# matthieugomez/LeastSquaresOptim.jl

Measured on AMD Instinct MI355X. Metric: lm_lsmr_outer_iterations_per_sec, higher is better.
Workload: dtype f64

## Files before the change

include/lsqhip.h:

```cpp
#ifndef LSQHIP_H
#define LSQHIP_H
#include <stddef.h>
#ifdef __cplusplus
extern "C" {
#endif

typedef enum {
    LSQ_OK = 0,
    LSQ_EDIM = 1,
    LSQ_ENOTPD = 2,
    LSQ_ERANK = 3,
    LSQ_ENONFINITE = 4,
    LSQ_EBOUNDS = 5,
    LSQ_EHIP = 6,
    LSQ_EARG = 7,
    LSQ_ECALLBACK = 8,
    LSQ_ERCCL = 9
} lsq_status;

typedef struct lsq_ctx lsq_ctx;
typedef struct lsq_mat lsq_mat;
typedef struct lsq_solver lsq_solver;
typedef struct lsq_model lsq_model;

// ... 128 lines not shown
    int bad_index;
    double seconds;
    long long lsmr_iterations;
    double ssr0;
} lsq_result;

void lsq_options_default(lsq_options *opt);
int lsq_optimize(lsq_ctx *ctx, int optimizer, int solver_kind, lsq_mat *J, double *d_x,
                 double *d_fcur, lsq_f_callback f, lsq_g_callback g, void *user,
                 const lsq_options *opt, lsq_result *res);

typedef struct {
    double *ssr, *ssr0;
    int *iterations;
    int *converged, *x_converged, *f_converged, *g_converged;
    int *f_calls, *g_calls, *mul_calls;
    int *status, *info;
    int outer_iterations;
    double seconds;
    int trace_cap;
    double *trace_ssr, *trace_gnorm, *trace_delta, *trace_rho;
    int *trace_accept;
    double *trace_x;
} lsq_batched_result;
int lsq_optimize_batched(lsq_ctx *ctx, int optimizer, int solver_kind, lsq_mat *J, double *d_x,
                         double *d_fcur, lsq_f_callback f, lsq_g_callback g, void *user,
                         const lsq_options *opt, void *batched_result);

int lsq_model_tanh_create(lsq_ctx *ctx, lsq_mat *J, const double *h_Avalues, const double *h_b,
                          lsq_model **out);
int lsq_model_destroy(lsq_model *md);
lsq_f_callback lsq_model_f(void);
lsq_g_callback lsq_model_g(void);

int lsq_synth_sparse(int m, int n, int per_col, unsigned long long seed, int *h_colptr,
                     int *h_rowval, double *h_nzval);
int lsq_synth_dense(int m, int n, unsigned long long seed, double *h_values);
int lsq_synth_uniform(int n, unsigned long long seed, double lo, double hi, double *h_out);
int lsq_synth_normal(int n, unsigned long long seed, double *h_out);

int lsq_bench_mul(lsq_mat *J, int trans, int reps, const double *d_x, double *d_y, double beta,
                  float *h_ms_per_launch);

int lsq_bench_occupy(lsq_ctx *ctx, int workgroups, int lds_bytes, double milliseconds);
int lsq_bench_occupy_wait(lsq_ctx *ctx);

int lsq_set_exact(int on);

int lsq_debug_set(int launch_jitter_us, int serial);
int lsq_debug_get(int *launch_jitter_us, int *serial, long long *stalls);

int lsq_prof_begin(lsq_ctx *ctx, int max_samples);
int lsq_prof_select(lsq_ctx *ctx, int kernel_mask);
int lsq_prof_end(lsq_ctx *ctx, double h_avg_ms[2], int h_count[2]);
int lsq_prof_overhead(lsq_ctx *ctx, int pairs, double *h_ms);

#ifdef __cplusplus
}
#endif
#endif
```

leastsquaresoptim.jl_amd/_lib.py:

```python
import ctypes as C
import os
import re
import subprocess

_HERE = os.path.dirname(os.path.abspath(__file__))
ROOT = os.path.dirname(_HERE)
LIB_PATH = os.environ.get("LSQ_LIB_PATH") or os.path.join(_HERE, "liblsqhip.so")
HEADER = os.path.join(ROOT, "include", "lsqhip.h")

c_dp = C.POINTER(C.c_double)
c_ip = C.POINTER(C.c_int)

F_CALLBACK = C.CFUNCTYPE(C.c_int, C.c_void_p, C.c_void_p, C.c_void_p)
G_CALLBACK = C.CFUNCTYPE(C.c_int, C.c_void_p, C.c_void_p, C.c_void_p)
ALLREDUCE_CALLBACK = C.CFUNCTYPE(C.c_int, c_dp, C.c_int, C.c_void_p)
OP_MUL_CALLBACK = C.CFUNCTYPE(C.c_int, C.c_int, C.c_void_p, C.c_void_p, C.c_void_p)
OP_COLSUM_CALLBACK = C.CFUNCTYPE(C.c_int, C.c_void_p, C.c_void_p)
PRECOND_CALLBACK = C.CFUNCTYPE(C.c_int, C.c_void_p, C.c_void_p, C.c_void_p, C.c_void_p)
ROW_ALLREDUCE_CALLBACK = C.CFUNCTYPE(C.c_int, C.c_void_p, C.c_int, C.c_void_p, C.c_void_p)
PRECOND_UPDATE_CALLBACK = C.CFUNCTYPE(C.c_int, C.c_void_p, C.c_void_p, C.c_void_p)
PRECOND_LDIV_CALLBACK = C.CFUNCTYPE(C.c_int, C.c_void_p, C.c_void_p, C.c_void_p)

OK, EDIM, ENOTPD, ERANK, ENONFINITE, EBOUNDS, EHIP, EARG, ECALLBACK, ERCCL = range(10)
QR, CHOLESKY, LSMR, BLOCK_QR = 0, 1, 2, 3
# ... 113 lines not shown
        "lsq_clamp": (i, [vp, i, d, d, vp]),
        "lsq_ediv": (i, [vp, i, vp, vp, vp]),
        "lsq_box_clip": (i, [vp, i, vp, vp, vp, vp]),
        "lsq_first_nonfinite": (i, [vp, i, vp, c_ip]),
        "lsq_solver_create": (i, [vp, vp, i, i, pvp]),
        "lsq_solver_destroy": (i, [vp]),
        "lsq_ldiv": (i, [vp, vp, vp, vp, c_ip]),
        "lsq_ldiv_damped": (i, [vp, vp, vp, vp, vp, c_ip]),
        "lsq_solver_set_row_allreduce": (i, [vp, ROW_ALLREDUCE_CALLBACK, vp, C.c_longlong]),
        "lsq_solver_info": (i, [vp, c_ip, c_ip, c_ip]),
        "lsq_solver_qr_path": (i, [vp, c_ip]),
        "lsq_solver_qr_panel": (i, [vp, c_ip]),
        "lsq_solver_chol_path": (i, [vp, c_ip]),
        "lsq_solver_lsmr_path": (i, [vp, c_ip]),
        "lsq_solver_blockdiag_path": (i, [vp, c_ip, c_ip]),
        "lsq_solver_blockdiag_ranks": (i, [vp, c_ip]),
        "lsq_solver_covariance": (i, [vp, vp, vp, vp, vp, c_ip]),
        "lsq_dense_covariance": (i, [vp, vp, vp, vp, vp, c_ip]),
        "lsq_solver_stats": (i, [vp, c_ip, c_ip]),
        "lsq_ctx_fallback_stats": (i, [vp, c_ip]),
        "lsq_ctx_device_info": (i, [vp, c_ip, c_ip, C.c_char_p, i]),
        "lsq_ctx_tail_stats": (i, [vp, C.POINTER(C.c_longlong)]),
        "lsq_bench_occupy": (i, [vp, i, i, d]),
        "lsq_bench_occupy_wait": (i, [vp]),
        "lsq_options_default": (None, [C.POINTER(Options)]),
        "lsq_optimize": (i, [vp, i, i, vp, vp, vp, F_CALLBACK, G_CALLBACK, vp, C.POINTER(Options),
                             C.POINTER(Result)]),
        "lsq_optimize_batched": (i, [vp, i, i, vp, vp, vp, F_CALLBACK, G_CALLBACK, vp, C.POINTER(Options),
                                     C.POINTER(BatchedResult)]),
        "lsq_model_tanh_create": (i, [vp, vp, c_dp, c_dp, pvp]),
        "lsq_model_destroy": (i, [vp]),
        "lsq_model_f": (F_CALLBACK, []),
        "lsq_model_g": (G_CALLBACK, []),
        "lsq_synth_sparse": (i, [i, i, i, C.c_ulonglong, c_ip, c_ip, c_dp]),
        "lsq_synth_dense": (i, [i, i, C.c_ulonglong, c_dp]),
        "lsq_synth_uniform": (i, [i, C.c_ulonglong, d, d, c_dp]),
        "lsq_synth_normal": (i, [i, C.c_ulonglong, c_dp]),
        "lsq_set_exact": (i, [i]),
        "lsq_debug_set": (i, [i, i]),
        "lsq_debug_get": (i, [c_ip, c_ip, C.POINTER(C.c_longlong)]),
        "lsq_prof_begin": (i, [vp, i]),
        "lsq_prof_select": (i, [vp, i]),
        "lsq_prof_end": (i, [vp, c_dp, c_ip]),
        "lsq_prof_overhead": (i, [vp, i, c_dp]),
        "lsq_bench_mul": (i, [vp, i, i, vp, vp, d, C.POINTER(C.c_float)]),
    }
    for name, (res, args) in sig.items():
        fn = getattr(L, name)
        fn.restype = res
        fn.argtypes = args
    L._signatures = sig
    _LIB = L
    return L


class LsqError(RuntimeError):

    def __init__(self, status, msg):
        super().__init__(msg)
        self.status = status


class DimensionMismatch(LsqError):
    pass


# ... 34 lines not shown
```

leastsquaresoptim.jl_amd/csrc/lsq_optimize.hip:

```cpp
#include <chrono>
#include <cmath>
#include <cstring>

#include "lsq_solver.h"
#include "lsq_spmv.h"

static constexpr double MIN_DELTA = 1e-16, MAX_DELTA = 1e16, MIN_STEP_QUALITY = 1e-3;
static constexpr double MIN_DIAGONAL = 1e-6, MAX_DIAGONAL = 1e32;
static constexpr double DECREASE_THRESHOLD = 0.25, INCREASE_THRESHOLD = 0.75;

enum { SL_GRAD = 8, SL_DX = 9, SL_NONFIN = 10, SL_TRIAL = 11, SL_PRED = 12, SL_SSR = 13, SL_W0 = 14, SL_W1 = 15,
       SL_W2 = 16, SL_SUM = 17 };

extern "C" int lsq_solver_create(lsq_ctx *c, lsq_mat *J, int kind, int for_lm, lsq_solver **out) {
    LSQ_RANGE("lsq_solver_create");
    if (!c || !J || !out) return LSQ_EARG;
    if (kind == LSQ_QR && J->kind != LSQ_MAT_DENSE) {
        lsq_set_error("solver QR() is not available for sparse Jacobians. Choose between Cholesky() and LSMR()");
        return LSQ_EARG;
    }
    const bool blockdiag = kind == LSQ_CHOLESKY && J->kind == LSQ_MAT_CSC && J->bd_blocks > 0;
    const bool bordered = kind == LSQ_CHOLESKY && J->kind == LSQ_MAT_CSC && J->br_blocks > 0;
    if (kind == LSQ_CHOLESKY && J->kind != LSQ_MAT_DENSE && !blockdiag && !bordered) {
        lsq_set_error("MethodError: no AbstractAllocatedSolver for Cholesky() with a sparse Jacobian "
// ... 1155 lines not shown
            res->status = LSQ_EARG;
            return LSQ_EARG;
        }
        LSQ_TRY(lsq_solver_set_row_allreduce(w->solver, opt->row_allreduce, opt->row_allreduce_user,
                                             opt->global_rows > 0 ? opt->global_rows : (long long)J->m));
    } else if (w->solver->kind == LSQ_LSMR) {
        LSQ_TRY(lsq_solver_set_row_allreduce(w->solver, nullptr, nullptr, 0));
    }
    auto t0 = std::chrono::steady_clock::now();
    int st = lm ? optimize_lm(c, w->solver, *w->buf, J, x, fcur, f, g, user, opt, res)
                : optimize_dogleg(c, w->solver, *w->buf, J, x, fcur, f, g, user, opt, res);
    hipStreamSynchronize(c->stream);
    res->seconds = std::chrono::duration<double>(std::chrono::steady_clock::now() - t0).count();
    res->status = st;
    return st;
}

struct lsq_model {
    lsq_ctx *ctx;
    lsq_mat *J;
    bool fused = false;
    double *d_Acsc = nullptr;
    double *d_Acsr = nullptr;
    double *d_Ab = nullptr;
    double *d_b = nullptr;
    double *d_t = nullptr;
    double *d_s = nullptr;
    double *d_sspec = nullptr;
    const double *tanh_x = nullptr;
    const double *sfac_x = nullptr;
    double *d_b_perm = nullptr;
    double *d_perm[2] = {nullptr, nullptr};
    const double *perm_of[2] = {nullptr, nullptr};
};
static void model_perm_invalidate(lsq_model *md, const double *vec) {
    for (int k = 0; k < 2; ++k)
        if (!vec || md->perm_of[k] == vec) md->perm_of[k] = nullptr;
}

__global__ void __launch_bounds__(LSQ_NT) k_tanh(int n, const double *__restrict__ x, double *__restrict__ t) {
    for (int i = blockIdx.x * LSQ_NT + threadIdx.x; i < n; i += gridDim.x * LSQ_NT) t[i] = tanh(x[i]);
}

struct EpiResidual {
    static constexpr bool REDUCE = false;
    const int *done;
    int extra_blocks;
    const double *b;
    double *out;
    double *partials;
    unsigned *counter;
    __device__ void seg(int i, double dot, double &) const { out[i] = dot - b[i]; }
    using has_pre = void;
    __device__ double pre(int i) const { return b[i]; }
    __device__ void seg_pre(int i, double dot, double bi, double &) const { out[i] = dot - bi; }
    __device__ void extra(int, double &) const {}
    __device__ void finalize(double) const {}
};

struct EpiResidualSq {
    static constexpr bool REDUCE = true;
    const int *done;
    int extra_blocks;
    const double *b;
    double *out;
    double *partials;
// ... 230 lines not shown
    return hipGetLastError() == hipSuccess ? 0 : 1;
}

static int model_pair_tail(void *user, lsq_mat *J, const double *dx, const double *fcur, double *ftrial, const double *xt,
                           double *slot_pred, double *slot_trial, LsqSlotPublish pub, const int *skip, bool *done, SpecGrad *sg) {
    lsq_model *md = (lsq_model *)user;
    lsq_ctx *c = md->ctx;
    *done = false;
    if (!(model_pair_applies(md, J) && md->tanh_x == xt)) return 0;
    const LsqSell &S = J->srows;
    const int nxpad = (J->n + 1) & ~1;
    const size_t lds = (size_t)std::max(2 * nxpad, LSQ_SELL_ROWS_MAX) * sizeof(double);
    if (lsq_set_lds(c, (const void *)k_sell_rows_pair<0>, (size_t)2 * LSQ_PAIR_X_MAX * sizeof(double)) != LSQ_OK) return 0;
    const size_t plen = (size_t)S.nslices * 64;
    const int pgrid = std::max(1, std::min(lsq_div_up((long long)plen, LSQ_NT), c->num_cus * 8));
    if (!model_perm_ready(md)) return 0;
    int k = md->perm_of[0] == fcur ? 0 : (md->perm_of[1] == fcur ? 1 : -1);
    if (k < 0) {
        k = 0;
        LSQ_LAUNCH(k_sell_perm_rows<0>, dim3(pgrid), dim3(LSQ_NT), 0, c->stream, sell_dev(S), S.wrows, S.nslices, fcur, md->d_perm[k]);
        md->perm_of[k] = fcur;
    }
    md->perm_of[1 - k] = ftrial;
    md->tanh_x = nullptr;
    const int grid = std::max(1, std::min(S.nblocks, c->num_cus));
    const bool spec = sg && sg->gate && md->sfac_x == xt;
    SellPairEpi e{skip, md->d_perm[k], md->d_b_perm, ftrial, md->d_perm[1 - k], c->d_partials, c->d_partials + 4096, lsq_ctr(c, 7),
                  slot_pred, slot_trial, pub, spec ? sg->gate : nullptr, spec ? sg->ssr : 0.0, MIN_STEP_QUALITY,
                  c->d_slots + SL_SSR, c->d_slots + SL_DX, c->d_slots + SL_GRAD, spec ? sg->xtol : 0.0, spec ? sg->ftol : 0.0,
                  spec ? sg->gtol : 0.0};
    LSQ_LAUNCH(k_sell_rows_pair<0>, dim3(grid), dim3(LSQ_BIG_NT), lds, c->stream, sell_dev(S), S.wrows, J->m, dx, J->d_colscale,
               (const double *)md->d_t, J->n, nxpad, e);
    *done = true;
    if (hipGetLastError() != hipSuccess) return 1;
    if (spec) {
        const int st = lsq_sparse_grad_colsum_spec(J, ftrial, sg->grad, md->d_sspec, sg->gate);
        if (st == LSQ_OK) sg->launched = true;
        else if (st != LSQ_EARG) return 1;
    }
    return 0;
}

static int model_g(lsq_mat *J, const double *x, void *user) {
    lsq_model *md = (lsq_model *)user;
    lsq_ctx *c = md->ctx;
    if (J->kind == LSQ_MAT_DENSE) {}
    else if (md->sfac_x == x) std::swap(md->d_s, md->d_sspec);
    else LSQ_LAUNCH(k_sfac, dim3(ngrid(c, J->n)), dim3(LSQ_NT), 0, c->stream, J->n, x, md->d_s);
    md->sfac_x = nullptr;
    md->tanh_x = nullptr;
    if (md->fused) {
        if (lsq_mat_set_colscale(J, md->d_s) != LSQ_OK) return 1;
        return hipGetLastError() == hipSuccess ? 0 : 1;
    }
    if (J->kind == LSQ_MAT_CSC) {
        const bool have_cols = J->scols.active || J->nwin > 1;
        const unsigned short *rcol = J->srows.active ? J->srows.d_idx16 : J->csr.d_idx16;
        const unsigned short *ccol = J->scols.active ? J->scols.d_col16 : J->bcsc.d_col16;
        double *rval = J->srows.active ? J->srows.d_val : J->csr.d_val;
        double *cval = J->scols.active ? J->scols.d_val : J->bcsc.d_val;
        const long long rlen = lsq_mirror_rows_len(J), clen = lsq_mirror_cols_len(J);
        const bool lds_ok = J->n <= 12000 && J->nnz >= (1 << 20) && J->srows.ncw == 1;
        const bool lazy_csc = lds_ok && rcol && have_cols && ccol && lsq_can_fuse_grad_colsum(J);
        if (!lazy_csc) {
            int grid = J->n < c->num_cus * 16 ? (J->n > 0 ? J->n : 1) : c->num_cus * 16;
            LSQ_LAUNCH(k_scale_cols, dim3(grid), dim3(LSQ_NT), 0, c->stream, J->n, J->csc.d_ptr, 0, md->d_Acsc,
// ... 64 lines not shown
    LSQ_HIP(hipMalloc(&md->d_t, nb));
    LSQ_HIP(hipMalloc(&md->d_s, nb));
    LSQ_HIP(hipMalloc(&md->d_sspec, nb));
    if (lsq_colscale_fusable(J)) {
        LSQ_TRY(lsq_mat_set_values(J, hA));
        LSQ_TRY(lsq_fill(c, J->n, 1.0, md->d_s));
        LSQ_TRY(lsq_mat_set_colscale(J, md->d_s));
        md->fused = true;
        LSQ_HIP(hipStreamSynchronize(c->stream));
        *out = md;
        return LSQ_OK;
    }
    size_t vb = (size_t)(J->nnz + 8) * sizeof(double);
    LSQ_HIP(hipMalloc(&md->d_Acsc, vb));
    LSQ_ZERO(md->d_Acsc, 0, vb);
    LSQ_HIP(hipMemcpy(md->d_Acsc, hA, (size_t)J->nnz * sizeof(double), hipMemcpyHostToDevice));
    if (J->kind == LSQ_MAT_CSC) {
        const size_t rb = (size_t)(lsq_mirror_rows_len(J) + 1024) * sizeof(double);
        LSQ_HIP(hipMalloc(&md->d_Acsr, rb));
        LSQ_ZERO(md->d_Acsr, 0, rb);
        LSQ_TRY(lsq_mirror_rows(J, md->d_Acsc, md->d_Acsr));
        if (lsq_mirror_cols_len(J) > 0) {
            const size_t cbytes = (size_t)(lsq_mirror_cols_len(J) + 1024) * sizeof(double);
            LSQ_HIP(hipMalloc(&md->d_Ab, cbytes));
            LSQ_ZERO(md->d_Ab, 0, cbytes);
            LSQ_TRY(lsq_mirror_cols(J, md->d_Acsc, md->d_Ab));
        }
        LSQ_HIP(hipStreamSynchronize(c->stream));
    }
    *out = md;
    return LSQ_OK;
}

extern "C" int lsq_model_destroy(lsq_model *md) {
    if (!md) return LSQ_OK;
    hipStreamSynchronize(md->ctx->stream);
    if (md->fused && md->J) lsq_mat_set_colscale(md->J, nullptr);
    hipFree(md->d_Acsc); hipFree(md->d_Acsr); hipFree(md->d_Ab); hipFree(md->d_b); hipFree(md->d_t); hipFree(md->d_s); hipFree(md->d_sspec);
    hipFree(md->d_b_perm); hipFree(md->d_perm[0]); hipFree(md->d_perm[1]);
    delete md;
    return LSQ_OK;
}
```

leastsquaresoptim.jl_amd/csrc/lsq_sell.h:

```cpp
#pragma once

constexpr int LSQ_SELL_POS_BITS = 13;
constexpr unsigned LSQ_SELL_POS_MASK = (1u << LSQ_SELL_POS_BITS) - 1u;
constexpr int LSQ_SELL_ROWS_MAX = 4096;
constexpr int LSQ_SELL_CW_AUTO = 6;
constexpr int LSQ_SELL_CW_MAX = 32;
constexpr int LSQ_SELL_GROWS_MAX = 16384;
constexpr int LSQ_SELL_CCOLS_MAX = 2560;

struct SellDev {
    const int2 *smeta;
    const unsigned *info;
    const unsigned short *idx16;
    const double *val;
    int nblocks;
    int spw;
};

template <int U>
struct SellBatch {
    double2 a[U];
    unsigned c[U];
};
template <int U, bool CLAMP>
// ... 58 lines not shown
    const int np = L >> 1;
    SellTail tail;
    tail.a = 0.0;
    tail.c = 0;
    if (TAIL && (L & 1)) tail = sell_tail_load(vp, ip, L, lane);
    for (; p0 + 8 <= np; p0 += 8) {
        SellBatch<8> B;
        sell_batch_load<8, false>(B, vp, ip, p0, np);
        sell_batch_sum<8, false, SQ>(B, p0, np, len, xl, sum, sq);
    }
    const int rem = np - p0;
    if (rem > 4) {
        SellBatch<8> B;
        sell_batch_load<8, true>(B, vp, ip, p0, np);
        sell_batch_sum<8, true, SQ>(B, p0, np, len, xl, sum, sq);
    } else if (rem > 2) {
        SellBatch<4> B;
        sell_batch_load<4, true>(B, vp, ip, p0, np);
        sell_batch_sum<4, true, SQ>(B, p0, np, len, xl, sum, sq);
    } else if (rem > 0) {
        SellBatch<2> B;
        sell_batch_load<2, true>(B, vp, ip, p0, np);
        sell_batch_sum<2, true, SQ>(B, p0, np, len, xl, sum, sq);
    }
    if (TAIL && (L & 1)) sell_tail_sum<SQ>(tail, L, len, xl, sum, sq);
}

template <bool SQ>
__device__ __forceinline__ void sell_lane_sum(const double *__restrict__ vp, const unsigned short *__restrict__ ip, int L, int len,
                                              const double *xl, double &sum, double &sq, int lane) {
    sell_lane_sum_from<SQ>(vp, ip, 0, L, len, xl, sum, sq, lane);
}

struct SellSliceRef {
    int2 sm;
    unsigned inf;
};
__device__ __forceinline__ SellSliceRef sell_slice_ref(const SellDev &S, int s, int s1, int lane) {
    SellSliceRef r;
    r.sm = make_int2(0, 0);
    r.inf = LSQ_SELL_POS_MASK;
    if (s < s1) {
        r.sm = S.smeta[__builtin_amdgcn_readfirstlane(s)];
        r.inf = S.info[(size_t)s * 64 + lane];
    }
    return r;
}
struct SellNoSliceHook {
    __device__ __forceinline__ double pre(size_t) const { return 0.0; }
    __device__ __forceinline__ void post(size_t, double, double) const {}
};
template <bool SQ, class Out, class Hook = SellNoSliceHook>
__device__ __forceinline__ void sell_wave_slices(const SellDev &S, int s0, int s1, int wv, int lane, const double *xl, Out out,
                                                 Hook hook = Hook()) {
    constexpr int NW = LSQ_BIG_NT / 64;
    int s = s0 + wv;
    SellSliceRef A = sell_slice_ref(S, s, s1, lane);
    __syncthreads();
    for (; s < s1; s += NW) {
        const SellSliceRef a = A;
        A = sell_slice_ref(S, s + NW, s1, lane);
        const size_t oa = (size_t)a.sm.x + lane * 2;
        const unsigned pos = a.inf & LSQ_SELL_POS_MASK;
        const size_t pidx = (size_t)s * 64 + lane;
        const double hp = hook.pre(pidx);
        double sum = 0.0, sq = 0.0;
        sell_lane_sum<SQ>(S.val + oa, S.idx16 + oa, a.sm.y, (int)(a.inf >> LSQ_SELL_POS_BITS), xl, sum, sq, lane);
        if (pos != LSQ_SELL_POS_MASK) {
            out(pos, sum, sq);
            hook.post(pidx, sum, hp);
        }
    }
}
template <class Epi>
struct SellEpiSliceHook {
    const Epi &epi;
    __device__ __forceinline__ double pre(size_t pidx) const { return epi.slice_pre(pidx); }
    __device__ __forceinline__ void post(size_t pidx, double sum, double p) const { epi.slice_post(pidx, sum, p); }
};

template <class Epi>
__global__ void __launch_bounds__(LSQ_BIG_NT) k_sell_rows(SellDev S, int wrows, int m, const double *__restrict__ x,
                                                          const double *__restrict__ xscale, int nx, int nxpad, Epi epi) {
    extern __shared__ __attribute__((aligned(16))) double smem[];
    __shared__ double sh[LSQ_BIG_NT / 64];
    double *xl = smem;
    double *yw = smem + nxpad;
    const int tid = threadIdx.x, lane = tid & 63, wv = tid >> 6;
    constexpr int XR = (LSQ_LDS_X_MAX + LSQ_BIG_NT - 1) / LSQ_BIG_NT;
    double xr[XR];
#pragma unroll
    for (int q = 0; q < XR; ++q) xr[q] = x[min(tid + q * LSQ_BIG_NT, nx - 1)];
    if (xscale) {
        double sr[XR];
#pragma unroll
        for (int q = 0; q < XR; ++q) sr[q] = xscale[min(tid + q * LSQ_BIG_NT, nx - 1)];
#pragma unroll
        for (int q = 0; q < XR; ++q) xr[q] *= sr[q];
    }
    const int dflag = epi.done ? *epi.done : 0;

    if constexpr (EpiHasBlockPrepare<Epi>::value) epi.block_prepare();
    if constexpr (EpiHasPrepare<Epi>::value) epi.prepare();
#pragma unroll
    for (int q = 0; q < XR; ++q)
        if (tid + q * LSQ_BIG_NT < nx) xl[tid + q * LSQ_BIG_NT] = xr[q];
    if (dflag) return;
    constexpr int Q = LSQ_SELL_ROWS_MAX / LSQ_BIG_NT;
    double racc = 0.0;
    for (int w = blockIdx.x; w < S.nblocks; w += gridDim.x) {
        const int base = w * wrows, rows = min(wrows, m - base);
        const int s0 = w * S.spw, s1 = s0 + S.spw;
        double pre[Q];
        if constexpr (EpiHasPre<Epi>::value) {
#pragma unroll
            for (int q = 0; q < Q; ++q) pre[q] = epi.pre(base + min(tid + q * LSQ_BIG_NT, rows - 1));
        }
        if constexpr (EpiHasSliceOut<Epi>::value)
            sell_wave_slices<false>(S, s0, s1, wv, lane, xl, [&](unsigned pos, double sum, double) { yw[pos] = sum; },
                                    SellEpiSliceHook<Epi>{epi});
        else
            sell_wave_slices<false>(S, s0, s1, wv, lane, xl, [&](unsigned pos, double sum, double) { yw[pos] = sum; });
        __syncthreads();
#pragma unroll
        for (int q = 0; q < Q; ++q) {
            const int i = tid + q * LSQ_BIG_NT;
            if (i < rows) {
                if constexpr (EpiHasPre<Epi>::value) epi.seg_pre(base + i, yw[i], pre[q], racc);
                else epi.seg(base + i, yw[i], racc);
            }
        }
    }
    for (int e = blockIdx.x; e < epi.extra_blocks; e += gridDim.x)
        if (tid < LSQ_NT) epi.extra(e, racc);
    finish_block_nt<LSQ_BIG_NT>(epi, racc, sh);
}

template <int U, bool CLAMP>
__device__ __forceinline__ void sell_batch_sum2(SellBatch<U> &B, int p0, int np, int len, const double *xa, const double *xb,
                                                double &sa, double &sb) {
#pragma unroll
    for (int u = 0; u < U; ++u) {
        const unsigned i0 = B.c[u] & 0xffffu, i1 = B.c[u] >> 16;
        double a0 = B.a[u].x * xa[i0], a1 = B.a[u].y * xa[i1], b0 = B.a[u].x * xb[i0], b1 = B.a[u].y * xb[i1];
        asm volatile("" : "+v"(a0), "+v"(a1), "+v"(b0), "+v"(b1));
        const int j = 2 * (p0 + u);
        const bool pin = !CLAMP || p0 + u < np;
        const bool in0 = pin && j < len, in1 = pin && j + 1 < len;
        const double ta0 = sa + a0;
        sa = in0 ? ta0 : sa;
        const double ta1 = sa + a1;
        sa = in1 ? ta1 : sa;
        const double tb0 = sb + b0;
        sb = in0 ? tb0 : sb;
        const double tb1 = sb + b1;
        sb = in1 ? tb1 : sb;
    }
}
__device__ __forceinline__ void sell_lane_sum2(const double *__restrict__ vp, const unsigned short *__restrict__ ip, int L, int len,
                                               const double *xa, const double *xb, double &sa, double &sb, int lane) {
    const int np = L >> 1;
    int p0 = 0;
    SellTail tail;
    tail.a = 0.0;
// ... 237 lines not shown
                const unsigned pos = a[g].inf & LSQ_SELL_POS_MASK;
                const size_t oa = (size_t)a[g].sm.x + lane * 2;
                double sum = pos != LSQ_SELL_POS_MASK ? yw[pos] : 0.0, sq = 0.0;
                sell_lane_sum_from<false, false>(S.val + oa, S.idx16 + oa, 2, a[g].sm.y, (int)(a[g].inf >> LSQ_SELL_POS_BITS), xl, sum, sq, lane);
                if (pos != LSQ_SELL_POS_MASK) yw[pos] = sum;
            }
        }
        double pre[Q];
        if constexpr (EpiHasPre<Epi>::value) {
#pragma unroll
            for (int q = 0; q < Q; ++q) pre[q] = epi.pre(base + min(tid + q * LSQ_WIDE_NT, rows - 1));
        }
        __syncthreads();
#pragma unroll
        for (int q = 0; q < Q; ++q) {
            const int i = tid + q * LSQ_WIDE_NT;
            if (i < rows) {
                if constexpr (EpiHasPre<Epi>::value) epi.seg_pre(base + i, yw[i], pre[q], racc);
                else epi.seg(base + i, yw[i], racc);
            }
        }
    }
    for (int e = blockIdx.x; e < epi.extra_blocks; e += gridDim.x)
        if (tid < LSQ_NT) epi.extra(e, racc);
    finish_block_nt<LSQ_WIDE_NT>(epi, racc, sh);
}

template <int = 0>
__global__ void __launch_bounds__(LSQ_NT) k_sell_vmul(int n, const double *__restrict__ a, const double *__restrict__ b,
                                                      double *__restrict__ out) {
    for (int i = blockIdx.x * LSQ_NT + threadIdx.x; i < n; i += gridDim.x * LSQ_NT) out[i] = a[i] * b[i];
}

__device__ __forceinline__ void sell_cols_stage_y(int b, int ncb, int grows, int m, const double *__restrict__ y, double *yl, int tid) {
    constexpr int YR = LSQ_SELL_GROWS_MAX / LSQ_BIG_NT;
    const int gw = b / ncb, gbase = gw * grows, rows = min(grows, m - gbase);
    double yr[YR];
#pragma unroll
    for (int j = 0; j < YR; ++j) yr[j] = y[gbase + min(tid + j * LSQ_BIG_NT, rows - 1)];
#pragma unroll
    for (int j = 0; j < YR; ++j)
        if (tid + j * LSQ_BIG_NT < grows) yl[tid + j * LSQ_BIG_NT] = (tid + j * LSQ_BIG_NT < rows) ? yr[j] : 0.0;
}
__device__ __forceinline__ int sell_cols_wg() { return lsq_xcd_block((int)blockIdx.x, (int)gridDim.x); }
__device__ __forceinline__ int sell_cols_first(int nblocks) {
    const int per = (nblocks + (int)gridDim.x - 1) / (int)gridDim.x;
    return sell_cols_wg() * per;
}
template <bool SQ>
__device__ __forceinline__ void sell_cols_pass(const SellDev &S, int ncb, int ccols, int grows, int m, int n,
                                               const double *__restrict__ y, double *__restrict__ part, double *smem) {
    double *yl = smem;
    double *ow = smem + LSQ_SELL_GROWS_MAX;
    const int tid = threadIdx.x, lane = tid & 63, wv = tid >> 6;
    const int per = (S.nblocks + (int)gridDim.x - 1) / (int)gridDim.x;
    const int b0 = sell_cols_wg() * per, b1 = min(S.nblocks, b0 + per);
    for (int b = b0; b < b1; ++b) {
        const int gw = b / ncb, cb = b - gw * ncb;
        const int cbase = cb * ccols, cols = min(ccols, n - cbase);
        if (b != b0) {
            __syncthreads();
            if (gw != (b - 1) / ncb) sell_cols_stage_y(b, ncb, grows, m, y, yl, tid);
        }
        const int s0 = b * S.spw, s1 = s0 + S.spw;
        double *dst = part + (size_t)gw * (SQ ? 2 : 1) * n + cbase;
        sell_wave_slices<SQ>(S, s0, s1, wv, lane, yl, [&](unsigned pos, double sum, double sq) {
            ow[pos] = sum;
            if constexpr (SQ) dst[n + pos] = sq;
        });
        __syncthreads();
        for (int i = tid; i < cols; i += LSQ_BIG_NT) dst[i] = ow[i];
    }
}

template <bool SQ>
__global__ void __launch_bounds__(LSQ_BIG_NT) k_sell_cols(SellDev S, int ncb, int ccols, int grows, int m, int n,
                                                          const double *__restrict__ y, double *__restrict__ part,
                                                          const int *done) {
    extern __shared__ __attribute__((aligned(16))) double smem[];
    const int dflag = done ? *done : 0;
    if (sell_cols_first(S.nblocks) < S.nblocks) sell_cols_stage_y(sell_cols_first(S.nblocks), ncb, grows, m, y, smem, threadIdx.x);
    if (dflag) return;
    sell_cols_pass<SQ>(S, ncb, ccols, grows, m, n, y, part, smem);
}
```

leastsquaresoptim.jl_amd/synthetic.py:

```python
import ctypes as C

import numpy as np

from . import _lib
from ._lib import check, lib
from .api import (DeviceVector, LeastSquaresResult, _run_native, _run_native_batched, default_context)

BASE_SEED = 20260928


def sparse_inputs(m, n, per_col, seed):
    nnz = n * per_col
    colptr = np.zeros(n + 1, dtype=np.int32)
    rowval = np.zeros(nnz, dtype=np.int32)
    nzval = np.zeros(nnz)
    check(lib().lsq_synth_sparse(m, n, per_col, seed, colptr.ctypes.data_as(_lib.c_ip),
                                 rowval.ctypes.data_as(_lib.c_ip), nzval.ctypes.data_as(_lib.c_dp)))
    return colptr, rowval, nzval


def dense_inputs(m, n, seed):
    v = np.zeros(m * n)
    check(lib().lsq_synth_dense(m, n, seed, v.ctypes.data_as(_lib.c_dp)))
    return v
# ... 122 lines not shown
        st, res, tr = _run_native(self.ctx, optimizer_kind, solver_kind, Jd, self.x, self.fcur,
                                  self._fg[0], self._fg[1], self.model, x_tol, f_tol, g_tol,
                                  iterations, delta, None, None, trace, self.n, allreduce=allreduce,
                                  row_allreduce=row_allreduce, row_allreduce_user=row_allreduce_user, global_rows=global_rows)
        check(st)
        r = LeastSquaresResult()
        r.optimizer = "LevenbergMarquardt" if res.optimizer == _lib.LEVENBERG_MARQUARDT else "Dogleg"
        r.ssr, r.iterations = float(res.ssr), res.iterations
        r.converged = bool(res.converged)
        r.x_converged, r.f_converged, r.g_converged = bool(res.x_converged), bool(res.f_converged), bool(res.g_converged)
        r.x_tol, r.f_tol, r.g_tol = x_tol, f_tol, g_tol
        r.f_calls, r.g_calls, r.mul_calls = res.f_calls, res.g_calls, res.mul_calls
        r.seconds, r.lsmr_iterations = res.seconds, int(res.lsmr_iterations)
        r.trace = tr
        r.minimizer = self.x.get() if fetch_x else None
        return r

    def optimize_batched(self, optimizer_kind=_lib.LEVENBERG_MARQUARDT, solver_kind=_lib.CHOLESKY, x_tol=1e-8, f_tol=1e-8,
                         g_tol=1e-8, iterations=1000, delta=None, lower=None, upper=None, trace=False, fetch_x=True):
        if self.blockdiag is None:
            raise _lib.ArgumentError(_lib.EARG, "optimize_batched needs a problem built with blockdiag=(nblocks, mb, nb)")
        if self._fg is None:
            L = lib()
            self._Jd = _Handle(self.J)
            self._fg = (L.lsq_model_f(), L.lsq_model_g())
        name = "LevenbergMarquardt" if optimizer_kind == _lib.LEVENBERG_MARQUARDT else "Dogleg"
        st, r = _run_native_batched(self.ctx, optimizer_kind, solver_kind, self.J, self.blockdiag, self.x, self.fcur,
                                    self._fg[0], self._fg[1], self.model, x_tol, f_tol, g_tol, iterations, delta, lower, upper,
                                    trace, name)
        check(st)
        r.minimizer = self.x.get() if fetch_x else None
        return r

    def close(self):
        L = lib()
        if self.model:
            L.lsq_model_destroy(self.model)
            self.model = None
        if self.J:
            L.lsq_mat_destroy(self.J)
            self.J = None
```

Measured before the change: 4090.

## Stage SELL x/y vectors into LDS via async DMA and prefetch first slice head

The SELL row and column SpMV kernels now copy the dense input vector into LDS with global_load_lds async DMA when it is 16-byte aligned and unscaled, instead of staging it through registers. Each wave also prefetches its first slice's values and indices into registers before the block barrier, so global loads overlap the staging. The early-exit done flag is deferred into the slice loop. A lsq_model_paths introspection API with a pair-tail counter is added. This depends on low-level waitcnt builtins and adds register pressure from the head buffer.

```diff
diff --git a/include/lsqhip.h b/include/lsqhip.h
--- a/include/lsqhip.h
+++ b/include/lsqhip.h
@@ -184,6 +184,7 @@
 int lsq_model_destroy(lsq_model *md);
 lsq_f_callback lsq_model_f(void);
 lsq_g_callback lsq_model_g(void);
+int lsq_model_paths(const lsq_model *md, int *sliced_rows, int *sliced_cols, int *lsmr_path, long long *pair_tails);
 
 int lsq_synth_sparse(int m, int n, int per_col, unsigned long long seed, int *h_colptr,
                      int *h_rowval, double *h_nzval);
diff --git a/leastsquaresoptim.jl_amd/_lib.py b/leastsquaresoptim.jl_amd/_lib.py
--- a/leastsquaresoptim.jl_amd/_lib.py
+++ b/leastsquaresoptim.jl_amd/_lib.py
@@ -169,6 +169,7 @@
         "lsq_model_destroy": (i, [vp]),
         "lsq_model_f": (F_CALLBACK, []),
         "lsq_model_g": (G_CALLBACK, []),
+        "lsq_model_paths": (i, [vp, c_ip, c_ip, c_ip, C.POINTER(C.c_longlong)]),
         "lsq_synth_sparse": (i, [i, i, i, C.c_ulonglong, c_ip, c_ip, c_dp]),
         "lsq_synth_dense": (i, [i, i, C.c_ulonglong, c_dp]),
         "lsq_synth_uniform": (i, [i, C.c_ulonglong, d, d, c_dp]),
diff --git a/leastsquaresoptim.jl_amd/csrc/lsq_optimize.hip b/leastsquaresoptim.jl_amd/csrc/lsq_optimize.hip
--- a/leastsquaresoptim.jl_amd/csrc/lsq_optimize.hip
+++ b/leastsquaresoptim.jl_amd/csrc/lsq_optimize.hip
@@ -1211,6 +1211,7 @@
     double *d_b_perm = nullptr;
     double *d_perm[2] = {nullptr, nullptr};
     const double *perm_of[2] = {nullptr, nullptr};
+    long long pair_tails = 0;
 };
 static void model_perm_invalidate(lsq_model *md, const double *vec) {
     for (int k = 0; k < 2; ++k)
@@ -1507,6 +1508,7 @@
     LSQ_LAUNCH(k_sell_rows_pair<0>, dim3(grid), dim3(LSQ_BIG_NT), lds, c->stream, sell_dev(S), S.wrows, J->m, dx, J->d_colscale,
                (const double *)md->d_t, J->n, nxpad, e);
     *done = true;
+    ++md->pair_tails;
     if (hipGetLastError() != hipSuccess) return 1;
     if (spec) {
         const int st = lsq_sparse_grad_colsum_spec(J, ftrial, sg->grad, md->d_sspec, sg->gate);
@@ -1637,6 +1639,20 @@
     return LSQ_OK;
 }
 
+extern "C" int lsq_model_paths(const lsq_model *md, int *sliced_rows, int *sliced_cols, int *lsmr_path, long long *pair_tails) {
+    if (!md || !sliced_rows || !sliced_cols || !lsmr_path || !pair_tails) {
+        lsq_set_error("lsq_model_paths: null argument");
+        return LSQ_EARG;
+    }
+    const lsq_mat *J = md->J;
+    *sliced_rows = J->kind == LSQ_MAT_CSC && J->srows.active;
+    *sliced_cols = J->kind == LSQ_MAT_CSC && J->scols.active;
+    const LsqWorkspace *w = (const LsqWorkspace *)md->ctx->workspace;
+    *lsmr_path = w && w->J == J && w->solver ? w->solver->last_lsmr_path : 0;
+    *pair_tails = md->pair_tails;
+    return LSQ_OK;
+}
+
 extern "C" int lsq_model_destroy(lsq_model *md) {
     if (!md) return LSQ_OK;
     hipStreamSynchronize(md->ctx->stream);
diff --git a/leastsquaresoptim.jl_amd/csrc/lsq_sell.h b/leastsquaresoptim.jl_amd/csrc/lsq_sell.h
--- a/leastsquaresoptim.jl_amd/csrc/lsq_sell.h
+++ b/leastsquaresoptim.jl_amd/csrc/lsq_sell.h
@@ -114,6 +114,129 @@
     sell_lane_sum_from<SQ>(vp, ip, 0, L, len, xl, sum, sq, lane);
 }
 
+struct SellStageTail {
+    double v;
+    int at;
+};
+__device__ __forceinline__ bool sell_stage_dma_ok(const double *src) { return ((unsigned long long)src & 15ull) == 0ull; }
+__device__ __forceinline__ void sell_stage_wait() { __builtin_amdgcn_s_waitcnt(0x0F70); }
+template <int NQ>
+__device__ __forceinline__ SellStageTail sell_stage_dma(const double *__restrict__ src, double *lds, int count, int tid) {
+    typedef const __attribute__((address_space(1))) void *gptr_t;
+    typedef __attribute__((address_space(3))) void *lptr_t;
+    const int nch = count >> 1;
+#pragma unroll
+    for (int q = 0; q < NQ; ++q) {
+        const int ch = q * LSQ_BIG_NT + tid;
+        if (ch < nch) __builtin_amdgcn_global_load_lds((gptr_t)(src + 2 * ch), (lptr_t)(lds + 2 * ch), 16, 0, 0);
+    }
+    SellStageTail t;
+    t.v = 0.0;
+    t.at = -1;
+    if ((count & 1) && tid == 0) {
+        t.v = src[count - 1];
+        t.at = count - 1;
+    }
+    return t;
+}
+__device__ __forceinline__ void sell_stage_tail_write(const SellStageTail &t, double *lds) {
+    if (t.at >= 0) lds[t.at] = t.v;
+}
+
+struct SellHead {
+    double2 a0, a1, a2, a3, a4, a5, a6, a7;
+    unsigned c0, c1, c2, c3, c4, c5, c6, c7;
+    double ta;
+    unsigned tc;
+};
+template <int U>
+__device__ __forceinline__ void sell_head_put(SellHead &H, const SellBatch<U> &B) {
+    static_assert(U == 2 || U == 4 || U == 8, "head batch");
+    H.a0 = B.a[0]; H.c0 = B.c[0];
+    H.a1 = B.a[1]; H.c1 = B.c[1];
+    if constexpr (U >= 4) {
+        H.a2 = B.a[2]; H.c2 = B.c[2];
+        H.a3 = B.a[3]; H.c3 = B.c[3];
+    }
+    if constexpr (U >= 8) {
+        H.a4 = B.a[4]; H.c4 = B.c[4];
+        H.a5 = B.a[5]; H.c5 = B.c[5];
+        H.a6 = B.a[6]; H.c6 = B.c[6];
+        H.a7 = B.a[7]; H.c7 = B.c[7];
+    }
+}
+template <int U>
+__device__ __forceinline__ void sell_head_get(const SellHead &H, SellBatch<U> &B) {
+    B.a[0] = H.a0; B.c[0] = H.c0;
+    B.a[1] = H.a1; B.c[1] = H.c1;
+    if constexpr (U >= 4) {
+        B.a[2] = H.a2; B.c[2] = H.c2;
+        B.a[3] = H.a3; B.c[3] = H.c3;
+    }
+    if constexpr (U >= 8) {
+        B.a[4] = H.a4; B.c[4] = H.c4;
+        B.a[5] = H.a5; B.c[5] = H.c5;
+        B.a[6] = H.a6; B.c[6] = H.c6;
+        B.a[7] = H.a7; B.c[7] = H.c7;
+    }
+}
+__device__ __forceinline__ void sell_head_load(SellHead &H, const double *__restrict__ val, const unsigned short *__restrict__ idx,
+                                               int off, int L, int lane) {
+    typedef const __attribute__((address_space(1))) char *gchar_t;
+    typedef double __attribute__((ext_vector_type(2))) gd2_t;
+    const int np = L >> 1;
+    unsigned vo = 16u * (unsigned)lane, io = 4u * (unsigned)lane;
+    asm volatile("" : "+v"(vo), "+v"(io));
+    const char *vb = reinterpret_cast<const char *>(val + off);
+    const char *ib = reinterpret_cast<const char *>(idx + off);
+    H.ta = 0.0;
+    H.tc = 0u;
+    if (L & 1) {
+        unsigned long long vt = (unsigned long long)(vb + (size_t)np * 1024), it = (unsigned long long)(ib + (size_t)np * 256);
+        asm volatile("" : "+s"(vt), "+s"(it));
+        H.ta = *(const __attribute__((address_space(1))) double *)((gchar_t)vt + (vo >> 1));
+        H.tc = *(const __attribute__((address_space(1))) unsigned *)((gchar_t)it + ((io >> 1) & ~3u));
+    }
+    if (np > 0) {
+        SellBatch<8> B;
+#pragma unroll
+        for (int u = 0; u < 8; ++u) {
+            const size_t q = (size_t)min(u, np - 1);
+            unsigned long long vq = (unsigned long long)(vb + q * 1024), iq = (unsigned long long)(ib + q * 256);
+            asm volatile("" : "+s"(vq), "+s"(iq));
+            const gd2_t v = *(const __attribute__((address_space(1))) gd2_t *)((gchar_t)vq + vo);
+            B.a[u].x = v.x;
+            B.a[u].y = v.y;
+            B.c[u] = *(const __attribute__((address_space(1))) unsigned *)((gchar_t)iq + io);
+        }
+        sell_head_put<8>(H, B);
+    }
+}
+template <int U, bool SQ>
+__device__ __forceinline__ void sell_head_sum_n(const SellHead &H, int np, int len, const double *xl, double &sum, double &sq) {
+    SellBatch<U> B;
+    sell_head_get<U>(H, B);
+    sell_batch_sum<U, true, SQ>(B, 0, np, len, xl, sum, sq);
+}
+template <bool SQ>
+__device__ __forceinline__ void sell_lane_sum_head(const SellHead &H, const double *__restrict__ vp, const unsigned short *__restrict__ ip,
+                                                   int L, int len, const double *xl, double &sum, double &sq, int lane) {
+    const int np = L >> 1;
+    if (np > 4) sell_head_sum_n<8, SQ>(H, np, len, xl, sum, sq);
+    else if (np > 2) sell_head_sum_n<4, SQ>(H, np, len, xl, sum, sq);
+    else if (np > 0) sell_head_sum_n<2, SQ>(H, np, len, xl, sum, sq);
+    if (np > 8) sell_lane_sum_from<SQ, false>(vp, ip, 8, L, len, xl, sum, sq, lane);
+    if (L & 1) {
+        SellTail t;
+        t.a = H.ta;
+        t.c = (unsigned short)(H.tc >> (16 * (lane & 1)));
+        sell_tail_sum<SQ>(t, L, len, xl, sum, sq);
+    }
+}
+
+struct SellNoBeforeBarrier {
+    __device__ __forceinline__ void operator()() const {}
+};
 struct SellSliceRef {
     int2 sm;
     unsigned inf;
@@ -132,13 +255,46 @@
     __device__ __forceinline__ double pre(size_t) const { return 0.0; }
     __device__ __forceinline__ void post(size_t, double, double) const {}
 };
-template <bool SQ, class Out, class Hook = SellNoSliceHook>
-__device__ __forceinline__ void sell_wave_slices(const SellDev &S, int s0, int s1, int wv, int lane, const double *xl, Out out,
-                                                 Hook hook = Hook()) {
+template <bool SQ, class Out, class Hook = SellNoSliceHook, class Before = SellNoBeforeBarrier>
+__device__ __forceinline__ bool sell_wave_slices(const SellDev &S, int s0, int s1, int wv, int lane, const double *xl, Out out,
+                                                 Hook hook = Hook(), Before before_barrier = Before(), int stop = 0,
+                                                 bool have_first = false, SellSliceRef first = SellSliceRef()) {
     constexpr int NW = LSQ_BIG_NT / 64;
     int s = s0 + wv;
-    SellSliceRef A = sell_slice_ref(S, s, s1, lane);
+    SellSliceRef A;
+    A.sm = make_int2(0, 0);
+    A.inf = LSQ_SELL_POS_MASK;
+    if (!have_first) A = sell_slice_ref(S, s, s1, lane);
+    SellHead H;
+    double hp0 = 0.0;
+    const int2 smv = have_first ? first.sm : A.sm;
+    const int2 sm0 = make_int2(__builtin_amdgcn_readfirstlane(smv.x), __builtin_amdgcn_readfirstlane(smv.y));
+    if (s < s1) {
+        sell_head_load(H, S.val, S.idx16, sm0.x, sm0.y, lane);
+        hp0 = hook.pre((size_t)s * 64 + lane);
+    }
+    before_barrier();
     __syncthreads();
+    asm volatile("" : "+v"(stop));
+    if (stop) return true;
+    if (s < s1) {
+        SellSliceRef a;
+        a.sm = sm0;
+        unsigned inf1 = first.inf;
+        asm volatile("" : "+v"(inf1));
+        a.inf = have_first ? inf1 : A.inf;
+        A = sell_slice_ref(S, s + NW, s1, lane);
+        const size_t oa = (size_t)a.sm.x + lane * 2;
+        const unsigned pos = a.inf & LSQ_SELL_POS_MASK;
+        const size_t pidx = (size_t)s * 64 + lane;
+        double sum = 0.0, sq = 0.0;
+        sell_lane_sum_head<SQ>(H, S.val + oa, S.idx16 + oa, a.sm.y, (int)(a.inf >> LSQ_SELL_POS_BITS), xl, sum, sq, lane);
+        if (pos != LSQ_SELL_POS_MASK) {
+            out(pos, sum, sq);
+            hook.post(pidx, sum, hp0);
+        }
+        s += NW;
+    }
     for (; s < s1; s += NW) {
         const SellSliceRef a = A;
         A = sell_slice_ref(S, s + NW, s1, lane);
@@ -153,6 +309,7 @@
             hook.post(pidx, sum, hp);
         }
     }
+    return false;
 }
 template <class Epi>
 struct SellEpiSliceHook {
@@ -170,24 +327,44 @@
     double *yw = smem + nxpad;
     const int tid = threadIdx.x, lane = tid & 63, wv = tid >> 6;
     constexpr int XR = (LSQ_LDS_X_MAX + LSQ_BIG_NT - 1) / LSQ_BIG_NT;
-    double xr[XR];
-#pragma unroll
-    for (int q = 0; q < XR; ++q) xr[q] = x[min(tid + q * LSQ_BIG_NT, nx - 1)];
-    if (xscale) {
-        double sr[XR];
-#pragma unroll
-        for (int q = 0; q < XR; ++q) sr[q] = xscale[min(tid + q * LSQ_BIG_NT, nx - 1)];
-#pragma unroll
-        for (int q = 0; q < XR; ++q) xr[q] *= sr[q];
-    }
-    const int dflag = epi.done ? *epi.done : 0;
-
-    if constexpr (EpiHasBlockPrepare<Epi>::value) epi.block_prepare();
-    if constexpr (EpiHasPrepare<Epi>::value) epi.prepare();
-#pragma unroll
-    for (int q = 0; q < XR; ++q)
-        if (tid + q * LSQ_BIG_NT < nx) xl[tid + q * LSQ_BIG_NT] = xr[q];
-    if (dflag) return;
+    SellStageTail xtail;
+    xtail.v = 0.0;
+    xtail.at = -1;
+    const bool dma = !xscale && sell_stage_dma_ok(x);
+    const SellSliceRef ref0 = sell_slice_ref(S, (int)blockIdx.x * S.spw + wv, (int)blockIdx.x < S.nblocks ? ((int)blockIdx.x + 1) * S.spw : 0, lane);
+    int dflag;
+    if (dma) {
+        xtail = sell_stage_dma<(XR + 1) / 2>(x, xl, nx, tid);
+        dflag = epi.done ? *epi.done : 0;
+        if constexpr (EpiHasBlockPrepare<Epi>::value) epi.block_prepare();
+        if constexpr (EpiHasPrepare<Epi>::value) epi.prepare();
+    } else {
+        double xr[XR];
+#pragma unroll
+        for (int q = 0; q < XR; ++q) xr[q] = x[min(tid + q * LSQ_BIG_NT, nx - 1)];
+        if (xscale) {
+            double sr[XR];
+#pragma unroll
+            for (int q = 0; q < XR; ++q) sr[q] = xscale[min(tid + q * LSQ_BIG_NT, nx - 1)];
+#pragma unroll
+            for (int q = 0; q < XR; ++q) xr[q] *= sr[q];
+        }
+        dflag = epi.done ? *epi.done : 0;
+
+        if constexpr (EpiHasBlockPrepare<Epi>::value) epi.block_prepare();
+        if constexpr (EpiHasPrepare<Epi>::value) epi.prepare();
+#pragma unroll
+        for (int q = 0; q < XR; ++q)
+            if (tid + q * LSQ_BIG_NT < nx) xl[tid + q * LSQ_BIG_NT] = xr[q];
+        sell_stage_wait();
+    }
+    if ((int)blockIdx.x >= S.nblocks) {
+        sell_stage_wait();
+        int d = dflag;
+        asm volatile("" : "+v"(d));
+        if (d) return;
+    }
+    bool pending = dma;
     constexpr int Q = LSQ_SELL_ROWS_MAX / LSQ_BIG_NT;
     double racc = 0.0;
     for (int w = blockIdx.x; w < S.nblocks; w += gridDim.x) {
@@ -198,11 +375,20 @@
 #pragma unroll
             for (int q = 0; q < Q; ++q) pre[q] = epi.pre(base + min(tid + q * LSQ_BIG_NT, rows - 1));
         }
+        auto staged = [&]() {
+            sell_stage_tail_write(xtail, xl);
+            if (pending) sell_stage_wait();
+        };
+        bool stopped;
         if constexpr (EpiHasSliceOut<Epi>::value)
-            sell_wave_slices<false>(S, s0, s1, wv, lane, xl, [&](unsigned pos, double sum, double) { yw[pos] = sum; },
-                                    SellEpiSliceHook<Epi>{epi});
+            stopped = sell_wave_slices<false>(S, s0, s1, wv, lane, xl, [&](unsigned pos, double sum, double) { yw[pos] = sum; },
+                                              SellEpiSliceHook<Epi>{epi}, staged, dflag, w == (int)blockIdx.x, ref0);
         else
-            sell_wave_slices<false>(S, s0, s1, wv, lane, xl, [&](unsigned pos, double sum, double) { yw[pos] = sum; });
+            stopped = sell_wave_slices<false>(S, s0, s1, wv, lane, xl, [&](unsigned pos, double sum, double) { yw[pos] = sum; },
+                                              SellNoSliceHook(), staged, dflag, w == (int)blockIdx.x, ref0);
+        if (stopped) return;
+        xtail.at = -1;
+        pending = false;
         __syncthreads();
 #pragma unroll
         for (int q = 0; q < Q; ++q) {
@@ -212,6 +398,7 @@
                 else epi.seg(base + i, yw[i], racc);
             }
         }
+        sell_stage_wait();
     }
     for (int e = blockIdx.x; e < epi.extra_blocks; e += gridDim.x)
         if (tid < LSQ_NT) epi.extra(e, racc);
@@ -515,15 +702,31 @@
     for (int i = blockIdx.x * LSQ_NT + threadIdx.x; i < n; i += gridDim.x * LSQ_NT) out[i] = a[i] * b[i];
 }
 
-__device__ __forceinline__ void sell_cols_stage_y(int b, int ncb, int grows, int m, const double *__restrict__ y, double *yl, int tid) {
+__device__ __forceinline__ SellStageTail sell_cols_stage_y(int b, int ncb, int grows, int m, const double *__restrict__ y, double *yl,
+                                                          int tid) {
     constexpr int YR = LSQ_SELL_GROWS_MAX / LSQ_BIG_NT;
     const int gw = b / ncb, gbase = gw * grows, rows = min(grows, m - gbase);
+    SellStageTail t;
+    t.v = 0.0;
+    t.at = -1;
+    if (sell_stage_dma_ok(y + gbase)) {
+        if (rows < grows) {
+#pragma unroll
+            for (int j = 0; j < YR; ++j) {
+                const int i = tid + j * LSQ_BIG_NT;
+                if (i >= rows && i < grows) yl[i] = 0.0;
+            }
+        }
+        return sell_stage_dma<YR / 2>(y + gbase, yl, rows, tid);
+    }
     double yr[YR];
 #pragma unroll
     for (int j = 0; j < YR; ++j) yr[j] = y[gbase + min(tid + j * LSQ_BIG_NT, rows - 1)];
 #pragma unroll
     for (int j = 0; j < YR; ++j)
         if (tid + j * LSQ_BIG_NT < grows) yl[tid + j * LSQ_BIG_NT] = (tid + j * LSQ_BIG_NT < rows) ? yr[j] : 0.0;
+    sell_stage_wait();
+    return t;
 }
 __device__ __forceinline__ int sell_cols_wg() { return lsq_xcd_block((int)blockIdx.x, (int)gridDim.x); }
 __device__ __forceinline__ int sell_cols_first(int nblocks) {
@@ -532,7 +735,8 @@
 }
 template <bool SQ>
 __device__ __forceinline__ void sell_cols_pass(const SellDev &S, int ncb, int ccols, int grows, int m, int n,
-                                               const double *__restrict__ y, double *__restrict__ part, double *smem) {
+                                               const double *__restrict__ y, double *__restrict__ part, double *smem,
+                                               SellStageTail ytail, int dflag, const SellSliceRef &ref0) {
     double *yl = smem;
     double *ow = smem + LSQ_SELL_GROWS_MAX;
     const int tid = threadIdx.x, lane = tid & 63, wv = tid >> 6;
@@ -543,16 +747,22 @@
         const int cbase = cb * ccols, cols = min(ccols, n - cbase);
         if (b != b0) {
             __syncthreads();
-            if (gw != (b - 1) / ncb) sell_cols_stage_y(b, ncb, grows, m, y, yl, tid);
+            if (gw != (b - 1) / ncb) ytail = sell_cols_stage_y(b, ncb, grows, m, y, yl, tid);
         }
         const int s0 = b * S.spw, s1 = s0 + S.spw;
         double *dst = part + (size_t)gw * (SQ ? 2 : 1) * n + cbase;
-        sell_wave_slices<SQ>(S, s0, s1, wv, lane, yl, [&](unsigned pos, double sum, double sq) {
+        const bool stopped = sell_wave_slices<SQ>(S, s0, s1, wv, lane, yl, [&](unsigned pos, double sum, double sq) {
             ow[pos] = sum;
             if constexpr (SQ) dst[n + pos] = sq;
-        });
+        }, SellNoSliceHook(), [&]() {
+            sell_stage_tail_write(ytail, yl);
+            sell_stage_wait();
+        }, dflag, b == b0, ref0);
+        if (stopped) return;
+        ytail.at = -1;
         __syncthreads();
         for (int i = tid; i < cols; i += LSQ_BIG_NT) dst[i] = ow[i];
+        sell_stage_wait();
     }
 }
 
@@ -562,7 +772,17 @@
                                                           const int *done) {
     extern __shared__ __attribute__((aligned(16))) double smem[];
     const int dflag = done ? *done : 0;
-    if (sell_cols_first(S.nblocks) < S.nblocks) sell_cols_stage_y(sell_cols_first(S.nblocks), ncb, grows, m, y, smem, threadIdx.x);
-    if (dflag) return;
-    sell_cols_pass<SQ>(S, ncb, ccols, grows, m, n, y, part, smem);
-}
+    const int bf = sell_cols_first(S.nblocks);
+    const SellSliceRef ref0 = sell_slice_ref(S, bf * S.spw + (int)(threadIdx.x >> 6), bf < S.nblocks ? (bf + 1) * S.spw : 0, threadIdx.x & 63);
+    SellStageTail ytail;
+    ytail.v = 0.0;
+    ytail.at = -1;
+    if (sell_cols_first(S.nblocks) < S.nblocks)
+        ytail = sell_cols_stage_y(sell_cols_first(S.nblocks), ncb, grows, m, y, smem, threadIdx.x);
+    if (bf >= S.nblocks) {
+        int d = dflag;
+        asm volatile("" : "+v"(d));
+        if (d) return;
+    }
+    sell_cols_pass<SQ>(S, ncb, ccols, grows, m, n, y, part, smem, ytail, dflag, ref0);
+}
diff --git a/leastsquaresoptim.jl_amd/synthetic.py b/leastsquaresoptim.jl_amd/synthetic.py
--- a/leastsquaresoptim.jl_amd/synthetic.py
+++ b/leastsquaresoptim.jl_amd/synthetic.py
@@ -178,6 +178,12 @@
         r.minimizer = self.x.get() if fetch_x else None
         return r
 
+    def paths(self):
+        rows, cols, lpath, pairs = C.c_int(), C.c_int(), C.c_int(), C.c_longlong()
+        check(lib().lsq_model_paths(self.model, C.byref(rows), C.byref(cols), C.byref(lpath), C.byref(pairs)))
+        return dict(sliced_rows=bool(rows.value), sliced_cols=bool(cols.value), pair_tails=pairs.value,
+                    lsmr_path={0: None, 1: "reference-order", 2: "four-launch", 3: "three-launch", 4: "general"}[lpath.value])
+
     def close(self):
         L = lib()
         if self.model:
```

New measurement: 4166, median of 6. 1.9% higher.
